# torognes/swarm

Hardware: AMD Instinct MI355X
Metric: amplicons/sec clustered (d=1) (higher is better)
Workload: dtype u64; 1 GPU; 10000000 synthetic amplicons x 150 bp, d=1 (10000000 per GPU; the metric's own size; configs[1]: configs1); per_gpu_queries=10000000, db_amplicons=10000000, step=swa_d1_index_build + swa_d1_network_device (B1 seam), db and CSR resident in HBM, route=streaming (d1_stream.inc), build=local, neighbour_links=17077441

## Files before the change

### swarm_amd/csrc/d1.hip

```cpp
#include "swa_internal.h"

#include <algorithm>
#include <type_traits>
#include <cstdlib>
#include <memory>
#include <thread>

namespace {

constexpr int kWaves = 4;
constexpr int kThreads = kWaves * 64;
constexpr int kQueueCap = 128;
constexpr uint32_t kEmpty = SWA_NO_AMPLICON;
constexpr size_t kMaxZobristLds = 96 * 1024;

struct alignas(16) swa_task {
  uint64_t hash;
  uint32_t heavy;
  uint32_t code;
};

struct NetArgs {
  const uint64_t * seqs;
  const uint64_t * seq_off;
// ... 748 lines not shown
  PartPlan p{};
  p.total = std::max(1u, total_bits);
  p.levels = (p.total + max_bits - 1) / max_bits;
  for (uint32_t l = 0; l < p.levels; ++l) { p.bits[l] = p.total / p.levels + (l < p.total % p.levels ? 1u : 0u); }
  return p;
}

struct PartJob {
  uint32_t nidx = 1;
  const unsigned long long * in[kMaxIdx] = {};
  unsigned long long * buf[kMaxIdx][2] = {};
  const uint64_t * cstart0[kMaxIdx] = {};
  uint64_t cstride0[kMaxIdx] = {};
  const uint32_t * csize0[kMaxIdx] = {};
  uint32_t csize_cap = 0, chunks0 = 1;
  bool single0 = true;
  uint64_t max_records = 0, max_tiles0 = 0;
  uint64_t out_cap = 0;
  uint32_t bias = 0, top_bit = 32;
  uint32_t tile = 4096;
  bool hist0_done = false;
  PartPlan plan{};
  uint32_t * out32[kMaxIdx] = {};
  uint32_t * cnt[kMaxIdx] = {}; uint32_t * ctile[kMaxIdx] = {}; uint64_t * starts[kMaxIdx] = {}; uint32_t * partial[kMaxIdx] = {};
  uint32_t * total[kMaxIdx] = {};
  uint64_t starts_stride = 0;
  const unsigned long long * out[kMaxIdx] = {}; const uint64_t * bstart[kMaxIdx] = {};
  uint32_t buckets = 0;
  int last = 0;
};

static void part_scratch(const PartJob & j, uint64_t * cnt, uint64_t * ctile, uint64_t * starts_half, uint64_t * partial) {
  uint64_t chunks = j.chunks0, c_max = 0, t_max = 0, s_max = 0;
  bool single = j.single0;
  for (uint32_t l = 0; l < j.plan.levels; ++l) {
    const uint64_t tiles = (l == 0 ? j.max_tiles0 : j.max_records / j.tile + chunks + 1);
    c_max = std::max(c_max, (tiles << j.plan.bits[l]) + 2);
    t_max = std::max(t_max, chunks + 2 + tiles + 2);
    chunks = (single ? 1 : chunks) << j.plan.bits[l];
    single = false;
    s_max = std::max(s_max, chunks + 2);
  }
  *cnt = c_max; *ctile = t_max; *starts_half = s_max; *partial = c_max / kFlatChunk + 2;
}

struct ClearList { uint32_t * p[8]; uint64_t words[8]; uint32_t n; };
__global__ __launch_bounds__(256) void k_clear_many(const ClearList c) {
  for (uint32_t k = 0; k < c.n; ++k) {
    for (uint64_t i = (uint64_t)blockIdx.x * blockDim.x + threadIdx.x; i < c.words[k]; i += (uint64_t)gridDim.x * blockDim.x) { c.p[k][i] = 0u; }
  }
}
static void clear_add(ClearList & c, void * p, uint64_t bytes) {
  c.p[c.n] = static_cast<uint32_t *>(p); c.words[c.n] = bytes / 4; ++c.n;
}
static int clear_launch(swa_ctx * ctx, const ClearList & c) {
  uint64_t most = 0;
  for (uint32_t k = 0; k < c.n; ++k) { most = std::max(most, c.words[k]); }
  if (c.n == 0 || most == 0) { return SWA_OK; }
  hipLaunchKernelGGL(k_clear_many, dim3(grid_for(ctx, most, 256, 8)), dim3(256), 0, ctx->stream, c);
  SWA_HIP(ctx, hipGetLastError());
  return SWA_OK;
}

static int run_partition(swa_ctx * ctx, PartJob & j) {
  uint64_t chunks = j.chunks0;
  bool single = j.single0;
  uint32_t used_bits = 0;
  const int cu_grid = ctx->num_cus * 8;
  for (uint32_t l = 0; l < j.plan.levels; ++l) {
    const uint32_t bits = j.plan.bits[l];
    used_bits += bits;
    const bool wide = bits > kPartMaxBits;
    const bool hist_done = l == 0 && j.hist0_done;
    const bool low_halves = l + 1 == j.plan.levels && j.out32[0] != nullptr;
    const bool have_form = wide ? (j.tile == 4096 || (j.tile == 8192 && hist_done)) && !low_halves
                                : (j.tile == 2048 && !low_halves) || j.tile == 4096;
    if (!have_form) { return swa_fail_msg(ctx, SWA_E_ARG, "partition: no kernel for this tile and bin count"); }
    PartArgs a{};
    a.single_seg = single ? 1u : 0u; a.bits = bits; a.shift = j.top_bit - used_bits; a.bias = j.bias; a.tile = j.tile;
    a.span = (single && l == 0 && chunks > 1 && j.tile == 4096 && !wide && !hist_done) ? 1u : 0u;
    const uint64_t tiles = (l == 0 ? j.max_tiles0 : j.max_records / j.tile + chunks + 1);
    a.run_bits = tiles >= (uint64_t)cu_grid ? 4u : 0u;
    for (uint32_t i = 0; i < j.nidx; ++i) {
      PartIdx & p = a.p[i];
      p.in = l == 0 ? j.in[i] : j.buf[i][(l - 1) & 1u];
      p.out = j.buf[i][l & 1u];
      p.out32 = low_halves ? j.out32[i] : nullptr;
      p.out_cap = j.out_cap;
      p.cstart = l == 0 ? j.cstart0[i] : j.starts[i] + ((l - 1) & 1u) * j.starts_stride;
      p.cstride = l == 0 ? j.cstride0[i] : 0;
      p.csize = l == 0 ? j.csize0[i] : nullptr;
      p.csize_cap = j.csize_cap;
      p.chunks = (uint32_t)chunks;
      p.ctile = j.ctile[i]; p.cnt = j.cnt[i];
      p.tchunk = j.ctile[i] + chunks + 1; p.tchunk_cap = (uint32_t)std::min<uint64_t>(tiles + 1, 0xFFFFFFFFu);
      p.next_start = j.starts[i] + (l & 1u) * j.starts_stride;
      p.total = j.total[i];
    }
    const dim3 grid_t((unsigned)((std::min<uint64_t>(std::max<uint64_t>(tiles, 1), (uint64_t)cu_grid) + 7) & ~7ull), j.nidx);
    if (chunks > 2048) { hipLaunchKernelGGL(k_part_tiles<1024>, dim3(1, j.nidx), dim3(1024), 0, ctx->stream, a); }
    else { hipLaunchKernelGGL(k_part_tiles<256>, dim3(1, j.nidx), dim3(256), 0, ctx->stream, a); }
    if (hist_done) {  }
    else if (wide) { hipLaunchKernelGGL((k_part_hist<1024, kPartTileMax, 256>), grid_t, dim3(256), 0, ctx->stream, a); }
    else if (a.span != 0u) { hipLaunchKernelGGL((k_part_hist<512, kPartTileMax, 256, true>), grid_t, dim3(256), 0, ctx->stream, a); }
    else { hipLaunchKernelGGL((k_part_hist<512, kPartTileMax, 256>), grid_t, dim3(256), 0, ctx->stream, a); }
    FlatScanArgs f{};
    f.unit_bits = bits;
    for (uint32_t i = 0; i < j.nidx; ++i) { f.v[i] = j.cnt[i]; f.units[i] = j.ctile[i] + chunks; f.partial[i] = j.partial[i]; f.total[i] = j.total[i]; }
    const dim3 grid_f((unsigned)std::min<uint64_t>(((tiles << bits) + 1 + kFlatChunk - 1) / kFlatChunk, (uint64_t)cu_grid), j.nidx);
    hipLaunchKernelGGL(k_flat_sums, grid_f, dim3(256), 0, ctx->stream, f);
    hipLaunchKernelGGL(k_flat_apply, grid_f, dim3(256), 0, ctx->stream, f);
    if (wide && j.tile == 8192) {
      constexpr size_t lds = part_scatter_lds(8192, 1024);
      if (!ctx->part_lds_opt_in) {
        SWA_HIP(ctx, hipFuncSetAttribute(reinterpret_cast<const void *>(&k_part_scatter<0, 8192, 1024, 1024>), hipFuncAttributeMaxDynamicSharedMemorySize, (int)lds));
        ctx->part_lds_opt_in = true;
      }
      hipLaunchKernelGGL((k_part_scatter<0, 8192, 1024, 1024>), grid_t, dim3(1024), lds, ctx->stream, a);
    }
    else if (wide) { hipLaunchKernelGGL((k_part_scatter<0, 4096, 1024, 512>), grid_t, dim3(512), part_scatter_lds(4096, 1024), ctx->stream, a); }
    else if (j.tile == 2048) { hipLaunchKernelGGL((k_part_scatter<0, 2048, 512, 512>), grid_t, dim3(512), part_scatter_lds(2048, 512), ctx->stream, a); }
    else if (a.span != 0u && low_halves) { hipLaunchKernelGGL((k_part_scatter<2, 4096, 512, 512, true>), grid_t, dim3(512), part_scatter_lds(4096, 512), ctx->stream, a); }
    else if (a.span != 0u) { hipLaunchKernelGGL((k_part_scatter<0, 4096, 512, 512, true>), grid_t, dim3(512), part_scatter_lds(4096, 512), ctx->stream, a); }
    else if (low_halves) { hipLaunchKernelGGL((k_part_scatter<2, 4096, 512, 512>), grid_t, dim3(512), part_scatter_lds(4096, 512), ctx->stream, a); }
    else { hipLaunchKernelGGL((k_part_scatter<0, 4096, 512, 512>), grid_t, dim3(512), part_scatter_lds(4096, 512), ctx->stream, a); }
    chunks = (single ? 1 : chunks) << bits;
    single = false;
    hipLaunchKernelGGL(k_part_starts, dim3((unsigned)std::min<uint64_t>((chunks + 256) / 256, (uint64_t)cu_grid), j.nidx), dim3(256), 0, ctx->stream, a);
    SWA_HIP(ctx, hipGetLastError());
  }
  j.buckets = (uint32_t)chunks;
  j.last = (int)((j.plan.levels - 1) & 1u);
  for (uint32_t i = 0; i < j.nidx; ++i) {
    j.out[i] = j.buf[i][j.last];
    j.bstart[i] = j.starts[i] + (uint64_t)j.last * j.starts_stride;
  }
  return SWA_OK;
}

static int ensure_lines(swa_ctx * ctx) {
  const uint32_t lq = line_quads_for(ctx);
  if (ctx->lines_ready && ctx->lines_quads == lq) { return SWA_OK; }
  const uint32_t n = ctx->db.n;
  SWA_TRY(swa_reserve(ctx, ctx->d_stream[kSbLines], (uint64_t)n * lq * 16u + 64u));
  auto * lines = static_cast<uint4 *>(ctx->d_stream[kSbLines].ptr);
  const auto * rank = static_cast<const uint32_t *>(ctx->d_arank.ptr);
  SWA_HIP(ctx, hipMemsetAsync(reinterpret_cast<uint8_t *>(lines) + (uint64_t)n * lq * 16u, 0, 64, ctx->stream));
  swa_t0(ctx, 15);
  const dim3 grid(grid_for(ctx, n, 256, 8));
  if (lq == 4u) { hipLaunchKernelGGL(k_lines_build<4>, grid, dim3(256), 0, ctx->stream, ctx->db.seqs, ctx->db.seq_off, ctx->db.seqlen, rank, n, lines); }
  else if (lq == 8u) { hipLaunchKernelGGL(k_lines_build<8>, grid, dim3(256), 0, ctx->stream, ctx->db.seqs, ctx->db.seq_off, ctx->db.seqlen, rank, n, lines); }
// ... 18 lines not shown
  const uint32_t lq = ctx->lines_quads;
  uint64_t item_room = 0;
  const ListRegions regions = list_regions(ctx, &item_room);
  const bool by_rec = ctx->route_rec[0] != nullptr;
  const bool routed = ctx->route_ids[0] != nullptr || by_rec;
  const uint64_t records = routed ? std::max<uint64_t>(std::max(ctx->route_m[0], ctx->route_m[1]), 1) : n;
  const uint32_t target = kG1Target, level_bits = 10u;
  uint32_t total_bits = 1;
  while ((records >> total_bits) > target && total_bits < 3 * kPartMaxBits) { ++total_bits; }
  total_bits = std::min<uint32_t>(total_bits + ctx->stream_extra_bits, 3 * kPartMaxBits);
  const bool keys_hist = !routed;
  PartJob j;
  j.nidx = 2;
  j.plan = total_bits <= level_bits ? plan_levels(total_bits, level_bits) : plan_levels(total_bits);
  j.max_records = records;
  j.out_cap = records + 1;
  const bool one_wide_level = total_bits > kPartMaxBits && j.plan.levels == 1;
  j.tile = one_wide_level ? (keys_hist ? 8192 : 4096) : 2048;
  j.max_tiles0 = records / j.tile + 2;
  j.chunks0 = 1; j.single0 = true; j.top_bit = 32; j.bias = 0;
  uint64_t e_cnt, e_tile, e_start, e_partial;
  part_scratch(j, &e_cnt, &e_tile, &e_start, &e_partial);
  const uint64_t buckets = 1ull << total_bits;
  e_partial = std::max<uint64_t>(e_partial, ((uint64_t)kListsPerIndex * buckets + 1) / kFlatChunk + 2);
  for (int i = 0; i < 2; ++i) {
    for (int h = 0; h < 2; ++h) { SWA_TRY(swa_reserve(ctx, ctx->d_stream[kSbRec + 2 * i + h], (records + 1) * sizeof(uint64_t))); }
    SWA_TRY(swa_reserve(ctx, ctx->d_stream[kSbCnt + i], e_cnt * sizeof(uint32_t)));
    SWA_TRY(swa_reserve(ctx, ctx->d_stream[kSbTile + i], e_tile * sizeof(uint32_t)));
    SWA_TRY(swa_reserve(ctx, ctx->d_stream[kSbStart + i], (2 * e_start + 4) * sizeof(uint64_t)));
    SWA_TRY(swa_reserve(ctx, ctx->d_stream[kSbPartial + i], e_partial * sizeof(uint32_t)));
    SWA_TRY(swa_reserve(ctx, ctx->d_stream[kSbMembers + i], (records + 1) * sizeof(uint32_t)));
    SWA_TRY(swa_reserve(ctx, ctx->d_stream[kSbKind + i], ((uint64_t)kListsPerIndex * buckets + 2) * sizeof(uint32_t)));
    SWA_TRY(swa_reserve(ctx, ctx->d_aitems[i], (item_room + 1) * sizeof(swa_item)));
  }
  SWA_TRY(swa_reserve(ctx, ctx->d_stream[kSbScal], 64 * sizeof(uint64_t)));
  SWA_TRY(swa_reserve(ctx, ctx->d_stream[kSbOver], ((uint64_t)n + 8) & ~3ull));
  SWA_TRY(swa_reserve(ctx, ctx->d_acounters, kCounterWords * sizeof(uint32_t)));
  {
    ClearList c{};
    clear_add(c, ctx->d_acounters.ptr, kCounterWords * sizeof(uint32_t));
    clear_add(c, ctx->d_guard.ptr, 8 * sizeof(uint64_t));
    clear_add(c, ctx->d_stream[kSbOver].ptr, ((uint64_t)n + 8) & ~3ull);
    for (int i = 0; i < 2; ++i) { clear_add(c, static_cast<uint32_t *>(ctx->d_stream[kSbKind + i].ptr) + (uint64_t)kListsPerIndex * buckets, sizeof(uint32_t)); }
    SWA_TRY(clear_launch(ctx, c));
  }
  swa_lap(ctx, "buffers reserved, counters cleared");
  auto * dflags = static_cast<uint32_t *>(ctx->d_flags.ptr);
  auto * scal = static_cast<uint64_t *>(ctx->d_stream[kSbScal].ptr);
  const uint32_t win_a = ctx->anchor_a, win_b = ctx->anchor_b;
  const uint32_t minlen = anchor_minlen(ctx), window_mode = (win_a != 0 || win_b != 0) ? 1u : 0u;

  KeyArgs k{};
  k.lines = static_cast<const uint4 *>(ctx->d_stream[kSbLines].ptr);
// ... 28 lines not shown
  else if (keys_hist) {
    const uint32_t ntiles = (uint32_t)((records + j.tile - 1) / j.tile);
    for (int i = 0; i < 2; ++i) { k.hist_cnt[i] = static_cast<uint32_t *>(ctx->d_stream[kSbCnt + i].ptr); }
    k.hist_bits = j.plan.bits[0]; k.hist_tile = j.tile; k.hist_ntiles = ntiles;
    k.hist_run_bits = j.max_tiles0 >= (uint64_t)ctx->num_cus * 8 ? 4u : 0u;
    const dim3 hgrid((unsigned)((std::min<uint64_t>(ntiles, (uint64_t)ctx->num_cus * 8) + 7) & ~7ull), 1u);
    hipLaunchKernelGGL(k_keys<true>, hgrid, dim3(256), 0, ctx->stream, k);
    j.hist0_done = true;
  } else {
    const dim3 kgrid((unsigned)grid_for(ctx, records, 256, 8), routed ? 2u : 1u);
    hipLaunchKernelGGL(k_keys<false>, kgrid, dim3(256), 0, ctx->stream, k);
  }
  swa_t1(ctx, 8);
  swa_lap(ctx, "k_keys");

  for (int i = 0; i < 2; ++i) {
    j.buf[i][0] = static_cast<unsigned long long *>(ctx->d_stream[kSbRec + 2 * i].ptr);
    j.buf[i][1] = static_cast<unsigned long long *>(ctx->d_stream[kSbRec + 2 * i + 1].ptr);
    j.in[i] = by_rec ? ctx->route_rec[i] : j.buf[i][1];
    j.cstart0[i] = nullptr; j.cstride0[i] = routed ? ctx->route_m[i] : n;
    j.cnt[i] = static_cast<uint32_t *>(ctx->d_stream[kSbCnt + i].ptr);
    j.ctile[i] = static_cast<uint32_t *>(ctx->d_stream[kSbTile + i].ptr);
    j.starts[i] = static_cast<uint64_t *>(ctx->d_stream[kSbStart + i].ptr);
    j.partial[i] = static_cast<uint32_t *>(ctx->d_stream[kSbPartial + i].ptr);
    j.total[i] = reinterpret_cast<uint32_t *>(scal + 8 + i);
  }
  j.starts_stride = e_start + 2;
  swa_t0(ctx, 9);
  SWA_TRY(run_partition(ctx, j));
  swa_t1(ctx, 9);
  swa_lap(ctx, "key partition");
  if (!ctx->guard_keys_done) {
    auto * gsum = static_cast<unsigned long long *>(ctx->d_guard.ptr) + 16;
    SWA_HIP(ctx, hipMemsetAsync(gsum, 0, 8 * sizeof(uint64_t), ctx->stream));
    GuardDbArgs gd{};
    gd.seqs = ctx->db.seqs; gd.seq_off = ctx->db.seq_off; gd.seqlen = ctx->db.seqlen; gd.n = n;
    for (int i = 0; i < 2; ++i) { gd.list[i] = k.list[i]; gd.list_count[i] = routed ? ctx->route_m[i] : 0; gd.list_rec[i] = by_rec ? ctx->route_rec[i] : nullptr; }
    gd.owner_rank = k.owner_rank; gd.owner_world = k.owner_world; gd.win_a = win_a; gd.win_b = win_b; gd.nwin = k.nwin;
    gd.out = gsum;
    hipLaunchKernelGGL(k_guard_db, dim3((unsigned)grid_for(ctx, records, 256, 8), routed ? 2u : 1u), dim3(256), 0, ctx->stream, gd);
    GuardRecArgs gr{};
    for (int i = 0; i < 2; ++i) { gr.rec[i] = j.out[i]; gr.total[i] = j.total[i]; }
    gr.out = gsum + 3;
    hipLaunchKernelGGL(k_guard_records, dim3((unsigned)grid_for(ctx, records, 256, 8), 2u), dim3(256), 0, ctx->stream, gr);
    ctx->guard_keys_pending = true;
  }

  swa_lap(ctx, "guard: second opinion");
  GroupArgs g{};
  for (int i = 0; i < 2; ++i) {
    GroupIdx & x = g.g[i];
    x.rec = const_cast<unsigned long long *>(j.out[i]);
    x.bstart = j.bstart[i];
    x.buckets = j.buckets;
    x.members = static_cast<uint32_t *>(ctx->d_stream[kSbMembers + i].ptr);
    x.items_tmp = j.buf[i][j.last ^ 1];
    x.kind_cnt = static_cast<uint32_t *>(ctx->d_stream[kSbKind + i].ptr);
  }
  g.pair_big = kPairBigCap; g.group_cap = kStreamGroupCap;
  g.flags = dflags;
  g.guard = static_cast<unsigned long long *>(ctx->d_guard.ptr);
  g.over = static_cast<uint8_t *>(ctx->d_stream[kSbOver].ptr);
  swa_t0(ctx, 10);
  {
    if (!ctx->g1_lds_opt_in) {
      SWA_HIP(ctx, hipFuncSetAttribute(reinterpret_cast<const void *>(&k_group1), hipFuncAttributeMaxDynamicSharedMemorySize, (int)kG1LdsBytes));
      ctx->g1_lds_opt_in = true;
    }
    hipLaunchKernelGGL(k_group1, dim3((unsigned)std::min<uint64_t>(buckets, (uint64_t)ctx->num_cus), 2), dim3(kG1Threads), kG1LdsBytes, ctx->stream, g);
  }
  swa_t1(ctx, 10);

  FlatScanArgs f{};
  ListArgs la{};
  auto * acounters = static_cast<uint32_t *>(ctx->d_acounters.ptr);
  for (int i = 0; i < 2; ++i) {
    f.v[i] = g.g[i].kind_cnt; f.units[i] = nullptr; f.fixed[i] = (uint64_t)kListsPerIndex * buckets + 1;
    f.partial[i] = j.partial[i]; f.total[i] = reinterpret_cast<uint32_t *>(scal + 10 + i);
    ListIdx & x = la.x[i];
    x.items_tmp = g.g[i].items_tmp; x.bstart = g.g[i].bstart; x.kind_pos = g.g[i].kind_cnt; x.buckets = (uint32_t)buckets;
    x.l.items = static_cast<swa_item *>(ctx->d_aitems[i].ptr);
    x.l.region = regions;
    x.l.counters = acounters + kCounterBase + (uint32_t)i * kWidthClasses * 8u;
    x.l.pair_big = g.pair_big;
  }
  const dim3 grid_k((unsigned)std::min<uint64_t>(((uint64_t)kListsPerIndex * buckets + kFlatChunk) / kFlatChunk, (uint64_t)ctx->num_cus * 8), 2);
  hipLaunchKernelGGL(k_flat_sums, grid_k, dim3(256), 0, ctx->stream, f);
  hipLaunchKernelGGL(k_flat_apply, grid_k, dim3(256), 0, ctx->stream, f);
  hipLaunchKernelGGL(k_group_lists, dim3((unsigned)std::min<uint64_t>((buckets + 3) / 4, (uint64_t)ctx->num_cus * 8), 2), dim3(256), 0, ctx->stream, la);
  SWA_HIP(ctx, hipGetLastError());
  swa_lap(ctx, "groups + work lists");
  ctx->list_regions_items = item_room;
  ctx->anchor_ready = true;
  ctx->stream_index = true;
  ctx->guard_index = true;
  return SWA_OK;
}

static int csr_from_chunks(swa_ctx * ctx, uint32_t first, uint32_t count, const unsigned long long * links, const uint64_t * d_cstart, uint64_t cstride,
                           const uint32_t * d_csize, uint32_t chunks, uint32_t csize_cap, uint64_t max_tiles0, uint64_t link_cap,
                           uint64_t * d_offsets, uint32_t * d_neighbours, uint64_t cap) {
  uint32_t nbits = 1;
  while (nbits < 32 && ((uint64_t)1 << nbits) < count) { ++nbits; }
  uint32_t r = std::min<uint32_t>(8, nbits - 1);
  if (nbits - r > 2 * kPartMaxBits) { r = std::min<uint32_t>(kCsrMaxR, nbits - 2 * kPartMaxBits); }
  PartJob j;
  j.nidx = 1;
  j.plan = plan_levels(nbits - r);
  j.max_records = link_cap;
  j.out_cap = link_cap;
  j.tile = 4096;
  j.max_tiles0 = max_tiles0;
  j.chunks0 = chunks; j.single0 = true; j.top_bit = nbits; j.bias = first;
  j.csize_cap = csize_cap;
  uint64_t e_cnt, e_tile, e_start, e_partial;
  part_scratch(j, &e_cnt, &e_tile, &e_start, &e_partial);
  SWA_TRY(swa_reserve(ctx, ctx->d_stream[kSbLinkA], (link_cap + 1) * sizeof(uint64_t)));
  SWA_TRY(swa_reserve(ctx, ctx->d_stream[kSbLinkB], (link_cap + 1) * sizeof(uint64_t)));
  SWA_TRY(swa_reserve(ctx, ctx->d_stream[kSbCnt], e_cnt * sizeof(uint32_t)));
  SWA_TRY(swa_reserve(ctx, ctx->d_stream[kSbTile], e_tile * sizeof(uint32_t)));
  SWA_TRY(swa_reserve(ctx, ctx->d_stream[kSbStart], (2 * e_start + 4) * sizeof(uint64_t)));
  SWA_TRY(swa_reserve(ctx, ctx->d_stream[kSbPartial], e_partial * sizeof(uint32_t)));
  SWA_TRY(swa_reserve(ctx, ctx->d_stream[kSbScal], 64 * sizeof(uint64_t)));
  j.in[0] = links;
  j.buf[0][0] = static_cast<unsigned long long *>(ctx->d_stream[kSbLinkA].ptr);
  j.buf[0][1] = static_cast<unsigned long long *>(ctx->d_stream[kSbLinkB].ptr);
  j.cstart0[0] = d_cstart; j.cstride0[0] = cstride;
  j.csize0[0] = d_csize;
  j.cnt[0] = static_cast<uint32_t *>(ctx->d_stream[kSbCnt].ptr);
  j.ctile[0] = static_cast<uint32_t *>(ctx->d_stream[kSbTile].ptr);
  j.starts[0] = static_cast<uint64_t *>(ctx->d_stream[kSbStart].ptr);
  j.partial[0] = static_cast<uint32_t *>(ctx->d_stream[kSbPartial].ptr);
  auto * extra = static_cast<uint64_t *>(ctx->d_status.ptr) + 48;
  j.total[0] = reinterpret_cast<uint32_t *>(extra + 1);
  j.starts_stride = e_start + 2;
  swa_t0(ctx, 13);
  SWA_TRY(run_partition(ctx, j));
  swa_t1(ctx, 13);
  CsrArgs c{};
  c.links = j.out[0]; c.bstart = j.bstart[0]; c.buckets = j.buckets; c.r = r; c.first = first; c.count = count;
  c.offsets = d_offsets; c.neighbours = d_neighbours; c.cap = d_neighbours != nullptr ? cap : 0;
  SWA_TRY(swa_reserve(ctx, ctx->d_stream[kSbHeavy], ((uint64_t)j.buckets + 2) * sizeof(uint32_t)));
  c.heavy = static_cast<uint32_t *>(ctx->d_stream[kSbHeavy].ptr) + 1;
  c.heavy_count = static_cast<uint32_t *>(ctx->d_stream[kSbHeavy].ptr);
  c.end_copy = extra;
  SWA_HIP(ctx, hipMemsetAsync(c.heavy_count, 0, sizeof(uint32_t), ctx->stream));
  swa_t0(ctx, 14);
  static const int csr_per_cu[2] = {
    [] { int nb = 0; return hipOccupancyMaxActiveBlocksPerMultiprocessor(&nb, k_csr_bucket<8>, 256, 0) == hipSuccess && nb > 0 ? nb : 4; }(),
    [] { int nb = 0; return hipOccupancyMaxActiveBlocksPerMultiprocessor(&nb, k_csr_bucket<9>, 256, 0) == hipSuccess && nb > 0 ? nb : 4; }() };
  const dim3 cgrid((unsigned)std::min<uint64_t>(((uint64_t)j.buckets + 3) / 4, (uint64_t)ctx->num_cus * (uint64_t)csr_per_cu[r <= 8 ? 0 : 1]));
  if (r <= 8) { hipLaunchKernelGGL(k_csr_bucket<8>, cgrid, dim3(256), 0, ctx->stream, c); }
  else { hipLaunchKernelGGL(k_csr_bucket<9>, cgrid, dim3(256), 0, ctx->stream, c); }
  hipLaunchKernelGGL(k_csr_bucket_big, dim3((unsigned)ctx->num_cus * 4), dim3(256), 0, ctx->stream, c);
  swa_t1(ctx, 14);
// ... 581 lines not shown
                         nseg, ctx->seg_cap, static_cast<const unsigned long long *>(ctx->d_seg_base.ptr), d_edge_list, cap);
    } else {
      stream_link_cap = std::max<uint64_t>(std::max<uint64_t>(cap, stream_link_cap), 2ull * count + 1024);
      SWA_TRY(launch_csr_stream(ctx, first, count, nseg, stream_link_cap, d_offsets, d_neighbours, cap));
    }
    SWA_HIP(ctx, hipGetLastError());
    swa_t1(ctx, 4);
    auto * status = static_cast<uint64_t *>(ctx->h_status);
    SWA_HIP(ctx, hipMemcpyAsync(status, ctx->d_status.ptr, 64 * sizeof(uint64_t), hipMemcpyDeviceToHost, ctx->stream));
    uint32_t * unserved_at = reinterpret_cast<uint32_t *>(status + 64);
    *unserved_at = 0;
    if (check_unserved) {
      SWA_HIP(ctx, hipMemcpyAsync(unserved_at, static_cast<uint32_t *>(ctx->d_acounters.ptr) + 2, sizeof(uint32_t), hipMemcpyDeviceToHost, ctx->stream));
    }
    SWA_HIP(ctx, hipStreamSynchronize(ctx->stream));
    const uint32_t unserved = *unserved_at;
    const uint64_t * got = status + 8 + 8;
    const uint64_t * guard = status + 24;
    const uint32_t anchor_overflow = reinterpret_cast<const uint32_t *>(status)[2];
    const uint64_t csr_end = status[48];
    const uint32_t links_sorted = (uint32_t)status[49];
    const bool guarded = ctx->anchor_usable;
    n_edges = got[0];
    if (guarded && anchor_overflow != 0) {
      ctx->stream_extra_bits = std::min<uint32_t>(ctx->stream_extra_bits + 2, 8);
      ctx->anchor_ready = false;
      continue;
    }
    if (check_unserved && unserved != 0) {
      SWA_TRY(ensure_full_index(ctx));
      continue;
    }
    if (d_edge_list == nullptr && got[1] <= ctx->seg_cap && n_edges > stream_link_cap) {
      stream_link_cap = n_edges + 1024;
      continue;
    }
    if (got[1] <= ctx->seg_cap) {
      clean = true;
      if (guarded) { SWA_TRY(guard_check(ctx, guard, got)); }
      if (d_edge_list == nullptr) { SWA_TRY(csr_check(ctx, csr_end, links_sorted, n_edges)); }
      twins = guarded && reinterpret_cast<const uint32_t *>(status)[0] != 0u;
      break;
    }
    while (ctx->seg_cap < 2 * got[1]) { ctx->seg_cap <<= 1; }
  }
  if (!clean) {
// ... 565 lines not shown
```

### swarm_amd/csrc/d1_stream.inc

```

constexpr uint32_t kPartTileMax = 4096;
constexpr uint32_t kPartMaxBits = 9;
constexpr unsigned long long kRecAbsent = ~0ull;
constexpr uint32_t kMaxIdx = 2;
constexpr uint32_t kStreamGroupCap = 4096;

template <int LQ>
__global__ __launch_bounds__(256) void k_lines_build(const uint64_t * __restrict__ seqs, const uint64_t * __restrict__ seq_off,
                                                     const uint32_t * __restrict__ seqlen, const uint32_t * __restrict__ rank, uint32_t n,
                                                     uint4 * __restrict__ lines) {
  constexpr uint32_t C = 2u * LQ - 1u;
  for (uint32_t i = blockIdx.x * blockDim.x + threadIdx.x; i < n; i += gridDim.x * blockDim.x) {
    const uint32_t len = seqlen[i];
    const uint64_t * s = seqs + seq_off[i];
    const uint32_t nw = (len + 31u) >> 5;
    uint32_t d[4 * LQ];
    d[0] = len; d[1] = rank[i];
#pragma unroll
    for (uint32_t k = 0; k < C; ++k) {
      const uint64_t w = k < nw ? s[k] : 0ull;
      d[2 + 2 * k] = (uint32_t)w; d[3 + 2 * k] = (uint32_t)(w >> 32);
    }
#pragma unroll
    for (uint32_t q = 0; q < (uint32_t)LQ; ++q) { lines[(uint64_t)i * LQ + q] = make_uint4(d[4 * q], d[4 * q + 1], d[4 * q + 2], d[4 * q + 3]); }
// ... 234 lines not shown
__global__ __launch_bounds__(256) void k_guard_records(const GuardRecArgs a) {
  const uint32_t which = blockIdx.y, m = *a.total[which];
  unsigned long long sum = 0ull;
  for (uint32_t e = blockIdx.x * blockDim.x + threadIdx.x; e < m; e += gridDim.x * blockDim.x) { sum += mix64(a.rec[which][e]); }
  guard_reduce(sum, a.out + which);
}

struct PartIdx {
  const unsigned long long * in;
  unsigned long long * out;
  uint32_t * out32;
  uint64_t out_cap;
  const uint64_t * cstart;
  uint64_t cstride;
  const uint32_t * csize;
  uint32_t csize_cap;
  uint32_t chunks;
  uint32_t * ctile;
  uint32_t * tchunk;
  uint32_t tchunk_cap;
  uint32_t * cnt;
  uint64_t * next_start;
  uint32_t * total;
};
struct PartArgs {
  PartIdx p[kMaxIdx];
  uint32_t single_seg;
  uint32_t shift, bits;
  uint32_t bias;
  uint32_t tile;
  uint32_t run_bits;
  uint32_t span;
};

__device__ __forceinline__ uint32_t part_chunk_size(const PartIdx & p, uint32_t c) {
  if (p.csize != nullptr) { return min(p.csize[c], p.csize_cap); }
  return p.cstart != nullptr ? (uint32_t)(p.cstart[c + 1] - p.cstart[c]) : (uint32_t)p.cstride;
}

template <uint32_t THREADS> __device__ __forceinline__ uint64_t block_exclusive_scan_of(uint64_t v, uint64_t * smem, uint64_t & total);
template <uint32_t THREADS>
__global__ __launch_bounds__(THREADS) void k_part_tiles(const PartArgs a) {
  __shared__ uint64_t smem[THREADS / 64u];
  const PartIdx & p = a.p[blockIdx.y];
  uint64_t carry = 0;
  const bool tile_pow2 = (a.tile & (a.tile - 1u)) == 0u;
  const uint32_t tile_shift = 31u - (uint32_t)__clz((int)a.tile);
  for (uint32_t base = 0; base < p.chunks; base += 8u * THREADS) {
    uint32_t v[8];
    uint64_t mine = 0;
#pragma unroll
    for (uint32_t k = 0; k < 8u; ++k) {
      const uint32_t c = base + threadIdx.x * 8u + k;
      v[k] = c < p.chunks ? (a.span != 0u ? part_chunk_size(p, c) : (part_chunk_size(p, c) + a.tile - 1u) / a.tile) : 0u;
    }
#pragma unroll
    for (uint32_t k = 0; k < 8u; ++k) { mine += v[k]; }
    uint64_t total;
    uint64_t run = carry + block_exclusive_scan_of<THREADS>(mine, smem, total);
#pragma unroll
    for (uint32_t k = 0; k < 8u; ++k) {
      const uint32_t c = base + threadIdx.x * 8u + k;
      if (c < p.chunks) {
        p.ctile[c] = (uint32_t)run;
        if (v[k] != 0u && a.span != 0u) {
          const uint32_t r32 = (uint32_t)run;
          const uint32_t first = tile_pow2 ? (r32 + a.tile - 1u) >> tile_shift : (r32 + a.tile - 1u) / a.tile;
// ... 112 lines not shown
    const uint32_t t = xcd_tile(v, a.run_bits);
    if (t >= ntiles) { continue; }
    for (uint32_t b = threadIdx.x; b < bins; b += THREADS) { hist[b] = 0u; }
    PartTile tile{0u, 0u, 0ull};
    const auto count_one = [&](unsigned long long r) {
      if (r != kRecAbsent) { atomicAdd(&hist[(((uint32_t)(r >> 32) - a.bias) >> a.shift) & (bins - 1u)], 1u); }
    };
    if constexpr (SPAN) {
      (void)part_span<TILE / THREADS, THREADS>(p, a.tile, t, span, [&](uint32_t, uint64_t place) { count_one(p.in[place]); });
    } else {
      tile = part_tile(p, a.tile, t, sh);
#pragma unroll
      for (uint32_t k = 0; k < TILE / THREADS; ++k) {
        const uint32_t j = k * THREADS + threadIdx.x;
        if (j < tile.count) { count_one(p.in[tile.first + j]); }
      }
    }
    __syncthreads();
    for (uint32_t b = threadIdx.x; b < bins; b += THREADS) { p.cnt[part_flat(a, p, tile.c, t, b)] = hist[b]; }
    __syncthreads();
  }
}

constexpr uint32_t kFlatChunk = 4096;
constexpr uint32_t kFlatPer = kFlatChunk / 256u;
struct FlatScanArgs { uint32_t * v[kMaxIdx]; const uint32_t * units[kMaxIdx]; uint32_t unit_bits; uint64_t fixed[kMaxIdx]; uint32_t * partial[kMaxIdx]; uint32_t * total[kMaxIdx]; };
__device__ __forceinline__ uint64_t flat_length(const FlatScanArgs & a, uint32_t i) {
  return a.units[i] != nullptr ? ((uint64_t)*a.units[i] << a.unit_bits) + 1u : a.fixed[i];
}

__global__ __launch_bounds__(256) void k_flat_sums(const FlatScanArgs a) {
  __shared__ uint64_t smem[4];
  const uint32_t * v = a.v[blockIdx.y];
  const uint64_t m = flat_length(a, blockIdx.y);
  for (uint64_t blk = blockIdx.x; blk * kFlatChunk < m; blk += gridDim.x) {
    const uint64_t base = blk * kFlatChunk + (uint64_t)threadIdx.x * kFlatPer;
    uint64_t s = 0;
#pragma unroll
    for (uint32_t k = 0; k < kFlatPer; ++k) { if (base + k < m) { s += v[base + k]; } }
    uint64_t total;
    (void)block_exclusive_scan(s, smem, total);
    if (threadIdx.x == 0) { a.partial[blockIdx.y][blk] = (uint32_t)total; }
  }
}

__global__ __launch_bounds__(256) void k_flat_apply(const FlatScanArgs a) {
  __shared__ uint64_t smem[4];
  uint32_t * v = a.v[blockIdx.y];
  const uint64_t m = flat_length(a, blockIdx.y);
  const uint32_t * partial = a.partial[blockIdx.y];
  const uint64_t nblk = (m + kFlatChunk - 1) / kFlatChunk;
  for (uint64_t blk = blockIdx.x; blk < nblk; blk += gridDim.x) {
    uint64_t before = 0;
    for (uint64_t q = threadIdx.x; q < blk; q += 256u) { before += partial[q]; }
    uint64_t prefix;
    (void)block_exclusive_scan(before, smem, prefix);
    const uint64_t base = blk * kFlatChunk + (uint64_t)threadIdx.x * kFlatPer;
    uint32_t c[kFlatPer];
    uint64_t s = 0;
#pragma unroll
    for (uint32_t k = 0; k < kFlatPer; ++k) { c[k] = base + k < m ? v[base + k] : 0u; s += c[k]; }
    uint64_t total;
    uint64_t run = prefix + block_exclusive_scan(s, smem, total);
#pragma unroll
    for (uint32_t k = 0; k < kFlatPer; ++k) { if (base + k < m) { v[base + k] = (uint32_t)run; } run += c[k]; }
    if (blk + 1 == nblk && threadIdx.x == 0) { *a.total[blockIdx.y] = (uint32_t)(prefix + total); }
  }
}

template <uint32_t THREADS>
__device__ __forceinline__ uint64_t block_exclusive_scan_of(uint64_t v, uint64_t * smem, uint64_t & total) {
  const uint32_t lane = threadIdx.x & 63u, wave = threadIdx.x >> 6;
  uint64_t incl = v;
#pragma unroll
  for (unsigned d = 1; d < 64; d <<= 1) { const uint64_t t = swa_shfl_up_u64(incl, d); if (lane >= d) { incl += t; } }
  if (lane == 63u) { smem[wave] = incl; }
  __syncthreads();
  uint64_t wave_off = 0, tot = 0;
#pragma unroll
  for (uint32_t w = 0; w < THREADS / 64u; ++w) { const uint64_t x = smem[w]; wave_off += w < wave ? x : 0ull; tot += x; }
  __syncthreads();
  total = tot;
  return wave_off + incl - v;
}

template <int MODE, uint32_t TILE, uint32_t BINS, uint32_t THREADS, bool SPAN = false>
__global__ __launch_bounds__(THREADS) __attribute__((amdgpu_waves_per_eu(SPAN && THREADS == 512 ? 8 : 1))) void k_part_scatter(const PartArgs a) {
  constexpr uint32_t kPartPer = TILE / THREADS;
  extern __shared__ __attribute__((aligned(16))) unsigned long long part_lds[];
// ... 56 lines not shown
        stage[at] = rec[k];
      }
    }
    __syncthreads();
    const uint32_t present = lstart[bins - 1u] + hist[bins - 1u];
#pragma unroll
    for (uint32_t k = 0; k < kPartPer; ++k) {
      const uint32_t j = k * THREADS + threadIdx.x;
      if (j < present) {
        const unsigned long long r = stage[j];
        const uint32_t d = (((uint32_t)(r >> 32) - a.bias) >> a.shift) & (bins - 1u);
        const uint64_t g = (uint64_t)goff[d] + (j - lstart[d]);
        if (g < p.out_cap) {
          if (MODE == 2) { p.out32[g] = (uint32_t)r; } else { p.out[g] = r; }
        }
      }
    }
    __syncthreads();
  }
}

constexpr size_t part_scatter_lds(uint32_t tile, uint32_t bins) { return (size_t)tile * 8u + 3u * (size_t)bins * 4u; }

__global__ __launch_bounds__(256) void k_part_starts(const PartArgs a) {
  const PartIdx & p = a.p[blockIdx.y];
  const uint32_t segs = a.single_seg != 0u ? 1u : p.chunks;
  const uint64_t buckets = (uint64_t)segs << a.bits;
  for (uint64_t i = (uint64_t)blockIdx.x * blockDim.x + threadIdx.x; i <= buckets; i += (uint64_t)gridDim.x * blockDim.x) {
    if (i == buckets) { p.next_start[i] = *p.total; continue; }
    const uint32_t c = (uint32_t)(i >> a.bits), b = (uint32_t)i & ((1u << a.bits) - 1u);
    p.next_start[i] = p.cnt[a.single_seg != 0u ? (uint64_t)b * p.ctile[p.chunks] : ((uint64_t)p.ctile[c] << a.bits) + (uint64_t)b * (p.ctile[c + 1] - p.ctile[c])];
  }
}

struct GroupIdx {
  unsigned long long * rec;
  const uint64_t * bstart;
  uint32_t buckets;
  uint32_t * members;
  unsigned long long * items_tmp;
  uint32_t * kind_cnt;
};
struct GroupArgs {
  GroupIdx g[kMaxIdx];
  uint32_t pair_big, group_cap;
  uint32_t * flags;
  unsigned long long * guard;
  uint8_t * over;
};

constexpr uint32_t kG1Threads = 1024;
constexpr uint32_t kG1SlotBits = 13, kG1Slots = 1u << kG1SlotBits;
constexpr uint32_t kG1DupBits = 14, kG1DupSlots = 1u << kG1DupBits;
constexpr uint32_t kG1Target = 10240;
constexpr size_t kG1LdsBytes = kG1Slots * 4 * 2 + kG1DupSlots * 4;
static_assert(kG1Slots * 4 <= kG1DupSlots * 4, "the groups' places lie in the area behind the two tables");
constexpr uint32_t kG1OverBit = 0x80000000u;

constexpr uint32_t kG1Per = 8;
constexpr uint32_t kG1Tail = 2;

__device__ __forceinline__ uint32_t g1_size(uint32_t w) { return w & 0xFFFFu; }
__device__ __forceinline__ uint32_t g1_class(uint32_t w) {
  const uint32_t bits = (w >> 16) & 0x1Fu;
  return bits == 0u ? 0u : 31u - (uint32_t)__clz((int)bits);
}
__device__ __forceinline__ bool g1_over(uint32_t w, uint32_t cap) { return g1_size(w) > 1u && (g1_size(w) > cap || g1_class(w) >= kTooLong); }
__device__ __forceinline__ uint32_t g1_list(uint32_t w, uint32_t pair_big, uint32_t cap) {
  const uint32_t g = g1_size(w);
  if (g < 2u || g1_over(w, cap)) { return kListsPerIndex; }
  const uint32_t kind = g <= kSeedsPerItem ? pair_class(g) : (g <= pair_big ? kPairClasses : kPairClasses + 1u);
// ... 94 lines not shown
    if ((int)lane >= d) { x += up; }
  }
  const unsigned long long tot = lane_value64(x, 15);
  const unsigned long long before = wave == 0u ? 0ull : lane_value64(x, (int)wave - 1);
  __syncthreads();
  total = tot;
  return before + incl - v;
}

__global__ __launch_bounds__(kG1Threads) void k_group1(const GroupArgs a) {
  extern __shared__ uint32_t g1_lds[];
  uint32_t * tcnt = g1_lds;
  uint32_t * tkey = tcnt + kG1Slots;
  uint32_t * toff = tkey + kG1Slots + (kG1DupSlots - kG1Slots);
  uint32_t * staged = tkey;
  __shared__ uint32_t kcnt[kListsPerIndex], kbase[kListsPerIndex];
  __shared__ unsigned long long smem16[16];
  __shared__ uint32_t sh_fail;
  __shared__ uint32_t gsum[3];
  uint32_t * glist = tkey;
  const uint32_t which = blockIdx.y;
  const GroupIdx & g = a.g[which];
  if (threadIdx.x < 3u) { gsum[threadIdx.x] = 0u; }
  for (uint32_t b = blockIdx.x; b < g.buckets; b += gridDim.x) {
    uint32_t tid = threadIdx.x;
    asm volatile("" : "+v"(tid));
    const uint32_t lane = tid & 63u;
    const uint64_t start = g.bstart[b];
    const uint32_t c = (uint32_t)(g.bstart[b + 1] - start);
    if (c == 0u) {
      if (tid < kListsPerIndex) { g.kind_cnt[tid * g.buckets + b] = 0u; }
      continue;
    }
    if (c > 0xFFFEu) {
      for (uint32_t r = tid; r < c; r += kG1Threads) {
        const uint32_t id = (uint32_t)g.rec[start + r];
        g.members[start + r] = id;
        atomicOr(reinterpret_cast<unsigned int *>(a.over + (id & ~3u)), (1u << which) << (8u * (id & 3u)));
      }
      if (tid < kListsPerIndex) { g.kind_cnt[tid * g.buckets + b] = 0u; }
      if (tid == 0) { atomicOr(a.flags + 4, 1u); atomicAdd(a.flags + 5, c); atomicAdd(a.guard + 6u + which, (unsigned long long)c); }
      continue;
    }
    const uint32_t cap = a.group_cap;
    uint32_t rkey[kG1Per], rid[kG1Per];
    uint32_t here = 0u;
// ... 502 lines not shown
```

Before: 5.998 billion amplicons/s.

## Replace two-pass flat scan with single-pass decoupled look-back scan fused with bucket starts

Replaces the k_flat_sums + k_flat_apply pair with one k_flat_scan kernel. It takes chunk indices from an atomic counter, publishes aggregate and inclusive flags, and looks back across earlier chunks one wavefront at a time. The same kernel also writes the next-level bucket start offsets from LDS, so the separate k_part_starts launch is removed. Scan state is widened to 64-bit status words and zeroed inside the preceding kernels. A spin bound reports stalls through a status word that the host checks. This cuts kernel launches and a full re-read of the counts per partition level. The cost is inter-block spinning, which depends on forward progress, plus some extra complexity.

```diff
diff --git a/swarm_amd/csrc/d1.hip b/swarm_amd/csrc/d1.hip
--- a/swarm_amd/csrc/d1.hip
+++ b/swarm_amd/csrc/d1.hip
@@ -794,13 +794,17 @@
   bool hist0_done = false;
   PartPlan plan{};
   uint32_t * out32[kMaxIdx] = {};
-  uint32_t * cnt[kMaxIdx] = {}; uint32_t * ctile[kMaxIdx] = {}; uint64_t * starts[kMaxIdx] = {}; uint32_t * partial[kMaxIdx] = {};
+  uint32_t * cnt[kMaxIdx] = {}; uint32_t * ctile[kMaxIdx] = {}; uint64_t * starts[kMaxIdx] = {};
+  unsigned long long * partial[kMaxIdx] = {};
   uint32_t * total[kMaxIdx] = {};
   uint64_t starts_stride = 0;
   const unsigned long long * out[kMaxIdx] = {}; const uint64_t * bstart[kMaxIdx] = {};
   uint32_t buckets = 0;
   int last = 0;
 };
+
+constexpr uint32_t kScanStallWord = 50;
+static unsigned long long * scan_stall_word(swa_ctx * ctx) { return static_cast<unsigned long long *>(ctx->d_status.ptr) + kScanStallWord; }
 
 static void part_scratch(const PartJob & j, uint64_t * cnt, uint64_t * ctile, uint64_t * starts_half, uint64_t * partial) {
   uint64_t chunks = j.chunks0, c_max = 0, t_max = 0, s_max = 0;
@@ -813,7 +817,7 @@
     single = false;
     s_max = std::max(s_max, chunks + 2);
   }
-  *cnt = c_max; *ctile = t_max; *starts_half = s_max; *partial = c_max / kFlatChunk + 2;
+  *cnt = c_max; *ctile = t_max; *starts_half = s_max; *partial = flat_state_words(c_max);
 }
 
 struct ClearList { uint32_t * p[8]; uint64_t words[8]; uint32_t n; };
@@ -853,6 +857,7 @@
     a.span = (single && l == 0 && chunks > 1 && j.tile == 4096 && !wide && !hist_done) ? 1u : 0u;
     const uint64_t tiles = (l == 0 ? j.max_tiles0 : j.max_records / j.tile + chunks + 1);
     a.run_bits = tiles >= (uint64_t)cu_grid ? 4u : 0u;
+    a.scan_words = (uint32_t)flat_state_words((tiles << bits) + 1);
     for (uint32_t i = 0; i < j.nidx; ++i) {
       PartIdx & p = a.p[i];
       p.in = l == 0 ? j.in[i] : j.buf[i][(l - 1) & 1u];
@@ -868,6 +873,7 @@
       p.tchunk = j.ctile[i] + chunks + 1; p.tchunk_cap = (uint32_t)std::min<uint64_t>(tiles + 1, 0xFFFFFFFFu);
       p.next_start = j.starts[i] + (l & 1u) * j.starts_stride;
       p.total = j.total[i];
+      p.scan_state = j.partial[i];
     }
     const dim3 grid_t((unsigned)((std::min<uint64_t>(std::max<uint64_t>(tiles, 1), (uint64_t)cu_grid) + 7) & ~7ull), j.nidx);
     if (chunks > 2048) { hipLaunchKernelGGL(k_part_tiles<1024>, dim3(1, j.nidx), dim3(1024), 0, ctx->stream, a); }
@@ -877,11 +883,13 @@
     else if (a.span != 0u) { hipLaunchKernelGGL((k_part_hist<512, kPartTileMax, 256, true>), grid_t, dim3(256), 0, ctx->stream, a); }
     else { hipLaunchKernelGGL((k_part_hist<512, kPartTileMax, 256>), grid_t, dim3(256), 0, ctx->stream, a); }
     FlatScanArgs f{};
-    f.unit_bits = bits;
-    for (uint32_t i = 0; i < j.nidx; ++i) { f.v[i] = j.cnt[i]; f.units[i] = j.ctile[i] + chunks; f.partial[i] = j.partial[i]; f.total[i] = j.total[i]; }
+    f.unit_bits = bits; f.single_seg = a.single_seg; f.stall = scan_stall_word(ctx);
+    for (uint32_t i = 0; i < j.nidx; ++i) {
+      f.v[i] = j.cnt[i]; f.units[i] = j.ctile[i] + chunks; f.partial[i] = j.partial[i]; f.total[i] = j.total[i];
+      f.next_start[i] = a.p[i].next_start; f.ctile[i] = j.ctile[i]; f.chunks[i] = (uint32_t)chunks;
+    }
     const dim3 grid_f((unsigned)std::min<uint64_t>(((tiles << bits) + 1 + kFlatChunk - 1) / kFlatChunk, (uint64_t)cu_grid), j.nidx);
-    hipLaunchKernelGGL(k_flat_sums, grid_f, dim3(256), 0, ctx->stream, f);
-    hipLaunchKernelGGL(k_flat_apply, grid_f, dim3(256), 0, ctx->stream, f);
+    hipLaunchKernelGGL(k_flat_scan, grid_f, dim3(kFlatThreads), 0, ctx->stream, f);
     if (wide && j.tile == 8192) {
       constexpr size_t lds = part_scatter_lds(8192, 1024);
       if (!ctx->part_lds_opt_in) {
@@ -898,7 +906,6 @@
     else { hipLaunchKernelGGL((k_part_scatter<0, 4096, 512, 512>), grid_t, dim3(512), part_scatter_lds(4096, 512), ctx->stream, a); }
     chunks = (single ? 1 : chunks) << bits;
     single = false;
-    hipLaunchKernelGGL(k_part_starts, dim3((unsigned)std::min<uint64_t>((chunks + 256) / 256, (uint64_t)cu_grid), j.nidx), dim3(256), 0, ctx->stream, a);
     SWA_HIP(ctx, hipGetLastError());
   }
   j.buckets = (uint32_t)chunks;
@@ -963,13 +970,13 @@
   uint64_t e_cnt, e_tile, e_start, e_partial;
   part_scratch(j, &e_cnt, &e_tile, &e_start, &e_partial);
   const uint64_t buckets = 1ull << total_bits;
-  e_partial = std::max<uint64_t>(e_partial, ((uint64_t)kListsPerIndex * buckets + 1) / kFlatChunk + 2);
+  e_partial = std::max<uint64_t>(e_partial, flat_state_words((uint64_t)kListsPerIndex * buckets + 1));
   for (int i = 0; i < 2; ++i) {
     for (int h = 0; h < 2; ++h) { SWA_TRY(swa_reserve(ctx, ctx->d_stream[kSbRec + 2 * i + h], (records + 1) * sizeof(uint64_t))); }
     SWA_TRY(swa_reserve(ctx, ctx->d_stream[kSbCnt + i], e_cnt * sizeof(uint32_t)));
     SWA_TRY(swa_reserve(ctx, ctx->d_stream[kSbTile + i], e_tile * sizeof(uint32_t)));
     SWA_TRY(swa_reserve(ctx, ctx->d_stream[kSbStart + i], (2 * e_start + 4) * sizeof(uint64_t)));
-    SWA_TRY(swa_reserve(ctx, ctx->d_stream[kSbPartial + i], e_partial * sizeof(uint32_t)));
+    SWA_TRY(swa_reserve(ctx, ctx->d_stream[kSbPartial + i], e_partial * sizeof(uint64_t)));
     SWA_TRY(swa_reserve(ctx, ctx->d_stream[kSbMembers + i], (records + 1) * sizeof(uint32_t)));
     SWA_TRY(swa_reserve(ctx, ctx->d_stream[kSbKind + i], ((uint64_t)kListsPerIndex * buckets + 2) * sizeof(uint32_t)));
     SWA_TRY(swa_reserve(ctx, ctx->d_aitems[i], (item_room + 1) * sizeof(swa_item)));
@@ -1044,7 +1051,7 @@
     j.cnt[i] = static_cast<uint32_t *>(ctx->d_stream[kSbCnt + i].ptr);
     j.ctile[i] = static_cast<uint32_t *>(ctx->d_stream[kSbTile + i].ptr);
     j.starts[i] = static_cast<uint64_t *>(ctx->d_stream[kSbStart + i].ptr);
-    j.partial[i] = static_cast<uint32_t *>(ctx->d_stream[kSbPartial + i].ptr);
+    j.partial[i] = static_cast<unsigned long long *>(ctx->d_stream[kSbPartial + i].ptr);
     j.total[i] = reinterpret_cast<uint32_t *>(scal + 8 + i);
   }
   j.starts_stride = e_start + 2;
@@ -1078,7 +1085,9 @@
     x.members = static_cast<uint32_t *>(ctx->d_stream[kSbMembers + i].ptr);
     x.items_tmp = j.buf[i][j.last ^ 1];
     x.kind_cnt = static_cast<uint32_t *>(ctx->d_stream[kSbKind + i].ptr);
-  }
+    x.scan_state = j.partial[i];
+  }
+  g.scan_words = (uint32_t)flat_state_words((uint64_t)kListsPerIndex * buckets + 1);
   g.pair_big = kPairBigCap; g.group_cap = kStreamGroupCap;
   g.flags = dflags;
   g.guard = static_cast<unsigned long long *>(ctx->d_guard.ptr);
@@ -1107,8 +1116,8 @@
     x.l.pair_big = g.pair_big;
   }
   const dim3 grid_k((unsigned)std::min<uint64_t>(((uint64_t)kListsPerIndex * buckets + kFlatChunk) / kFlatChunk, (uint64_t)ctx->num_cus * 8), 2);
-  hipLaunchKernelGGL(k_flat_sums, grid_k, dim3(256), 0, ctx->stream, f);
-  hipLaunchKernelGGL(k_flat_apply, grid_k, dim3(256), 0, ctx->stream, f);
+  f.stall = scan_stall_word(ctx);
+  hipLaunchKernelGGL(k_flat_scan, grid_k, dim3(kFlatThreads), 0, ctx->stream, f);
   hipLaunchKernelGGL(k_group_lists, dim3((unsigned)std::min<uint64_t>((buckets + 3) / 4, (uint64_t)ctx->num_cus * 8), 2), dim3(256), 0, ctx->stream, la);
   SWA_HIP(ctx, hipGetLastError());
   swa_lap(ctx, "groups + work lists");
@@ -1142,7 +1151,7 @@
   SWA_TRY(swa_reserve(ctx, ctx->d_stream[kSbCnt], e_cnt * sizeof(uint32_t)));
   SWA_TRY(swa_reserve(ctx, ctx->d_stream[kSbTile], e_tile * sizeof(uint32_t)));
   SWA_TRY(swa_reserve(ctx, ctx->d_stream[kSbStart], (2 * e_start + 4) * sizeof(uint64_t)));
-  SWA_TRY(swa_reserve(ctx, ctx->d_stream[kSbPartial], e_partial * sizeof(uint32_t)));
+  SWA_TRY(swa_reserve(ctx, ctx->d_stream[kSbPartial], e_partial * sizeof(uint64_t)));
   SWA_TRY(swa_reserve(ctx, ctx->d_stream[kSbScal], 64 * sizeof(uint64_t)));
   j.in[0] = links;
   j.buf[0][0] = static_cast<unsigned long long *>(ctx->d_stream[kSbLinkA].ptr);
@@ -1152,7 +1161,7 @@
   j.cnt[0] = static_cast<uint32_t *>(ctx->d_stream[kSbCnt].ptr);
   j.ctile[0] = static_cast<uint32_t *>(ctx->d_stream[kSbTile].ptr);
   j.starts[0] = static_cast<uint64_t *>(ctx->d_stream[kSbStart].ptr);
-  j.partial[0] = static_cast<uint32_t *>(ctx->d_stream[kSbPartial].ptr);
+  j.partial[0] = static_cast<unsigned long long *>(ctx->d_stream[kSbPartial].ptr);
   auto * extra = static_cast<uint64_t *>(ctx->d_status.ptr) + 48;
   j.total[0] = reinterpret_cast<uint32_t *>(extra + 1);
   j.starts_stride = e_start + 2;
@@ -1780,6 +1789,10 @@
     const uint32_t links_sorted = (uint32_t)status[49];
     const bool guarded = ctx->anchor_usable;
     n_edges = got[0];
+    if (status[kScanStallWord] != 0) {
+      SWA_HIP(ctx, hipMemsetAsync(scan_stall_word(ctx), 0, sizeof(uint64_t), ctx->stream));
+      return swa_fail_msg(ctx, SWA_E_INTERNAL, "d=1: a partition scan waited beyond its bound for the chunks before it");
+    }
     if (guarded && anchor_overflow != 0) {
       ctx->stream_extra_bits = std::min<uint32_t>(ctx->stream_extra_bits + 2, 8);
       ctx->anchor_ready = false;
diff --git a/swarm_amd/csrc/d1_stream.inc b/swarm_amd/csrc/d1_stream.inc
--- a/swarm_amd/csrc/d1_stream.inc
+++ b/swarm_amd/csrc/d1_stream.inc
@@ -280,6 +280,7 @@
   uint32_t * cnt;
   uint64_t * next_start;
   uint32_t * total;
+  unsigned long long * scan_state;
 };
 struct PartArgs {
   PartIdx p[kMaxIdx];
@@ -289,6 +290,7 @@
   uint32_t tile;
   uint32_t run_bits;
   uint32_t span;
+  uint32_t scan_words;
 };
 
 __device__ __forceinline__ uint32_t part_chunk_size(const PartIdx & p, uint32_t c) {
@@ -301,6 +303,7 @@
 __global__ __launch_bounds__(THREADS) void k_part_tiles(const PartArgs a) {
   __shared__ uint64_t smem[THREADS / 64u];
   const PartIdx & p = a.p[blockIdx.y];
+  for (uint32_t i = threadIdx.x; i < a.scan_words; i += THREADS) { p.scan_state[i] = 0ull; }
   uint64_t carry = 0;
   const bool tile_pow2 = (a.tile & (a.tile - 1u)) == 0u;
   const uint32_t tile_shift = 31u - (uint32_t)__clz((int)a.tile);
@@ -459,49 +462,132 @@
   }
 }
 
-constexpr uint32_t kFlatChunk = 4096;
-constexpr uint32_t kFlatPer = kFlatChunk / 256u;
-struct FlatScanArgs { uint32_t * v[kMaxIdx]; const uint32_t * units[kMaxIdx]; uint32_t unit_bits; uint64_t fixed[kMaxIdx]; uint32_t * partial[kMaxIdx]; uint32_t * total[kMaxIdx]; };
+constexpr uint32_t kFlatChunk = 8192;
+constexpr uint32_t kFlatThreads = 512;
+constexpr uint32_t kFlatPer = kFlatChunk / kFlatThreads;
+struct FlatScanArgs {
+  uint32_t * v[kMaxIdx]; const uint32_t * units[kMaxIdx]; uint32_t unit_bits; uint64_t fixed[kMaxIdx];
+  unsigned long long * partial[kMaxIdx];
+  uint32_t * total[kMaxIdx];
+  uint64_t * next_start[kMaxIdx]; const uint32_t * ctile[kMaxIdx]; uint32_t chunks[kMaxIdx]; uint32_t single_seg;
+  unsigned long long * stall;
+};
 __device__ __forceinline__ uint64_t flat_length(const FlatScanArgs & a, uint32_t i) {
   return a.units[i] != nullptr ? ((uint64_t)*a.units[i] << a.unit_bits) + 1u : a.fixed[i];
 }
-
-__global__ __launch_bounds__(256) void k_flat_sums(const FlatScanArgs a) {
-  __shared__ uint64_t smem[4];
-  const uint32_t * v = a.v[blockIdx.y];
-  const uint64_t m = flat_length(a, blockIdx.y);
-  for (uint64_t blk = blockIdx.x; blk * kFlatChunk < m; blk += gridDim.x) {
-    const uint64_t base = blk * kFlatChunk + (uint64_t)threadIdx.x * kFlatPer;
-    uint64_t s = 0;
-#pragma unroll
-    for (uint32_t k = 0; k < kFlatPer; ++k) { if (base + k < m) { s += v[base + k]; } }
-    uint64_t total;
-    (void)block_exclusive_scan(s, smem, total);
-    if (threadIdx.x == 0) { a.partial[blockIdx.y][blk] = (uint32_t)total; }
-  }
-}
-
-__global__ __launch_bounds__(256) void k_flat_apply(const FlatScanArgs a) {
-  __shared__ uint64_t smem[4];
-  uint32_t * v = a.v[blockIdx.y];
-  const uint64_t m = flat_length(a, blockIdx.y);
-  const uint32_t * partial = a.partial[blockIdx.y];
+constexpr uint64_t flat_state_words(uint64_t entries) { return (entries + kFlatChunk - 1) / kFlatChunk + 1; }
+
+typedef __attribute__((address_space(1))) unsigned long long flat_gu64;
+typedef __attribute__((address_space(1))) uint32_t flat_gu32;
+constexpr unsigned long long kScanAgg = 1ull << 32;
+constexpr unsigned long long kScanIncl = 2ull << 32;
+constexpr uint32_t kScanSpins = 1u << 22;
+
+__device__ __forceinline__ uint64_t flat_buckets_below(const FlatScanArgs & a, uint32_t y, uint64_t x) {
+  const uint32_t * ctile = a.ctile[y];
+  const uint32_t chunks = a.chunks[y], bits = a.unit_bits;
+  if (a.single_seg != 0u) {
+    const uint64_t tiles = ctile[chunks], most = (1ull << bits) + 1u;
+    if (tiles == 0u) { return x > 0u ? most : 0u; }
+    return min((x + tiles - 1u) / tiles, most);
+  }
+  const uint32_t lane = threadIdx.x & 63u;
+  uint32_t lo = 0, hi = chunks + 1u;
+  while (lo < hi) {
+    const uint32_t step = (hi - lo + 63u) / 64u, q = lo + (lane + 1u) * step - 1u;
+    const bool at_or_above = q < hi && ((uint64_t)ctile[q] << bits) >= x;
+    const unsigned long long m = __ballot(at_or_above);
+    if (m == 0ull) { lo += min(64u, (hi - lo) / step) * step; continue; }
+    const uint32_t k = (uint32_t)__ffsll((long long)m) - 1u;
+    hi = lo + (k + 1u) * step - 1u;
+    lo = k == 0u ? lo : lo + k * step;
+  }
+  if (lo == chunks + 1u) { return ((uint64_t)chunks << bits) + 1u; }
+  if (lo == 0u) { return 0u; }
+  const uint32_t c = lo - 1u, t0 = ctile[c], nt = ctile[lo] - t0;
+  const uint64_t first = (uint64_t)t0 << bits, all = 1ull << bits;
+  const uint64_t below = nt == 0u ? all : min(all, (x - first + nt - 1u) / nt);
+  return ((uint64_t)c << bits) + below;
+}
+
+__global__ __launch_bounds__(kFlatThreads) void k_flat_scan(const FlatScanArgs a) {
+  __shared__ uint64_t smem[kFlatThreads / 64u];
+  __shared__ uint32_t vals[kFlatChunk];
+  __shared__ uint64_t sh_range[2];
+  __shared__ uint32_t sh_blk, sh_prefix;
+  const uint32_t y = blockIdx.y, lane = threadIdx.x & 63u, wave = threadIdx.x >> 6;
+  uint32_t * v = a.v[y];
+  const uint64_t m = flat_length(a, y);
   const uint64_t nblk = (m + kFlatChunk - 1) / kFlatChunk;
-  for (uint64_t blk = blockIdx.x; blk < nblk; blk += gridDim.x) {
-    uint64_t before = 0;
-    for (uint64_t q = threadIdx.x; q < blk; q += 256u) { before += partial[q]; }
-    uint64_t prefix;
-    (void)block_exclusive_scan(before, smem, prefix);
-    const uint64_t base = blk * kFlatChunk + (uint64_t)threadIdx.x * kFlatPer;
+  flat_gu64 * status = (flat_gu64 *)(a.partial[y]) + 1;
+  const bool starts = a.next_start[y] != nullptr;
+  for (;;) {
+    if (threadIdx.x == 0) { sh_blk = __hip_atomic_fetch_add((flat_gu32 *)(a.partial[y]), 1u, __ATOMIC_RELAXED, __HIP_MEMORY_SCOPE_AGENT); }
+    __syncthreads();
+    const uint64_t blk = sh_blk;
+    if (blk >= nblk) { return; }
+    const uint64_t lo = blk * kFlatChunk, base = lo + (uint64_t)threadIdx.x * kFlatPer;
     uint32_t c[kFlatPer];
     uint64_t s = 0;
 #pragma unroll
     for (uint32_t k = 0; k < kFlatPer; ++k) { c[k] = base + k < m ? v[base + k] : 0u; s += c[k]; }
-    uint64_t total;
-    uint64_t run = prefix + block_exclusive_scan(s, smem, total);
-#pragma unroll
-    for (uint32_t k = 0; k < kFlatPer; ++k) { if (base + k < m) { v[base + k] = (uint32_t)run; } run += c[k]; }
-    if (blk + 1 == nblk && threadIdx.x == 0) { *a.total[blockIdx.y] = (uint32_t)(prefix + total); }
+    uint64_t agg;
+    const uint64_t run = block_exclusive_scan_of<kFlatThreads>(s, smem, agg);
+    if (wave == 0u) {
+      uint32_t prefix = 0;
+      if (blk == 0u) {
+        if (lane == 0u) { __hip_atomic_store(status, kScanIncl | (uint32_t)agg, __ATOMIC_RELAXED, __HIP_MEMORY_SCOPE_AGENT); }
+      } else {
+        if (lane == 0u) { __hip_atomic_store(status + blk, kScanAgg | (uint32_t)agg, __ATOMIC_RELAXED, __HIP_MEMORY_SCOPE_AGENT); }
+        int64_t end = (int64_t)blk - 1;
+        for (uint32_t spins = 0;;) {
+          const int64_t q = end - (int64_t)lane;
+          const unsigned long long w = q >= 0 ? __hip_atomic_load(status + q, __ATOMIC_RELAXED, __HIP_MEMORY_SCOPE_AGENT) : kScanIncl;
+          if (!__all((w >> 32) != 0ull)) {
+            if (++spins < kScanSpins) { __builtin_amdgcn_s_sleep(1); continue; }
+            if (lane == 0u) { atomicAdd(a.stall, 1ull); }
+            break;
+          }
+          const unsigned long long incl = __ballot((w >> 32) == 2ull);
+          const uint32_t upto = incl != 0ull ? (uint32_t)__ffsll((long long)incl) - 1u : 63u;
+          uint32_t x = lane <= upto ? (uint32_t)w : 0u;
+#pragma unroll
+          for (int o = 32; o > 0; o >>= 1) { x += (uint32_t)__shfl_xor((int)x, o, 64); }
+          prefix += x;
+          if (incl != 0ull) { break; }
+          end -= 64;
+        }
+        if (lane == 0u) { __hip_atomic_store(status + blk, kScanIncl | (uint32_t)(prefix + (uint32_t)agg), __ATOMIC_RELAXED, __HIP_MEMORY_SCOPE_AGENT); }
+      }
+      if (lane == 0u) { sh_prefix = prefix; }
+    } else if (starts && wave <= 2u) {
+      const uint64_t r = flat_buckets_below(a, y, wave == 1u ? lo : min(lo + kFlatChunk, m));
+      if (lane == 0u) { sh_range[wave - 1u] = r; }
+    }
+    __syncthreads();
+    uint32_t at = sh_prefix + (uint32_t)run;
+#pragma unroll
+    for (uint32_t k = 0; k < kFlatPer; ++k) {
+      if (base + k < m) { v[base + k] = at; }
+      if (starts) { vals[threadIdx.x * kFlatPer + k] = at; }
+      at += c[k];
+    }
+    if (blk + 1 == nblk && threadIdx.x == 0) { *a.total[y] = sh_prefix + (uint32_t)agg; }
+    if (starts) {
+      __syncthreads();
+      const uint32_t * ctile = a.ctile[y];
+      const uint32_t chunks = a.chunks[y], bits = a.unit_bits;
+      for (uint64_t i = sh_range[0] + threadIdx.x; i < sh_range[1]; i += kFlatThreads) {
+        uint64_t e;
+        if (a.single_seg != 0u) { e = i * ctile[chunks]; }
+        else {
+          const uint32_t cc = (uint32_t)(i >> bits), b = (uint32_t)i & ((1u << bits) - 1u);
+          e = cc == chunks ? (uint64_t)ctile[chunks] << bits : ((uint64_t)ctile[cc] << bits) + (uint64_t)b * (ctile[cc + 1] - ctile[cc]);
+        }
+        a.next_start[y][i] = vals[e - lo];
+      }
+    }
+    __syncthreads();
   }
 }
 
@@ -604,17 +690,6 @@
 
 constexpr size_t part_scatter_lds(uint32_t tile, uint32_t bins) { return (size_t)tile * 8u + 3u * (size_t)bins * 4u; }
 
-__global__ __launch_bounds__(256) void k_part_starts(const PartArgs a) {
-  const PartIdx & p = a.p[blockIdx.y];
-  const uint32_t segs = a.single_seg != 0u ? 1u : p.chunks;
-  const uint64_t buckets = (uint64_t)segs << a.bits;
-  for (uint64_t i = (uint64_t)blockIdx.x * blockDim.x + threadIdx.x; i <= buckets; i += (uint64_t)gridDim.x * blockDim.x) {
-    if (i == buckets) { p.next_start[i] = *p.total; continue; }
-    const uint32_t c = (uint32_t)(i >> a.bits), b = (uint32_t)i & ((1u << a.bits) - 1u);
-    p.next_start[i] = p.cnt[a.single_seg != 0u ? (uint64_t)b * p.ctile[p.chunks] : ((uint64_t)p.ctile[c] << a.bits) + (uint64_t)b * (p.ctile[c + 1] - p.ctile[c])];
-  }
-}
-
 struct GroupIdx {
   unsigned long long * rec;
   const uint64_t * bstart;
@@ -622,6 +697,7 @@
   uint32_t * members;
   unsigned long long * items_tmp;
   uint32_t * kind_cnt;
+  unsigned long long * scan_state;
 };
 struct GroupArgs {
   GroupIdx g[kMaxIdx];
@@ -629,6 +705,7 @@
   uint32_t * flags;
   unsigned long long * guard;
   uint8_t * over;
+  uint32_t scan_words;
 };
 
 constexpr uint32_t kG1Threads = 1024;
@@ -769,6 +846,7 @@
   const uint32_t which = blockIdx.y;
   const GroupIdx & g = a.g[which];
   if (threadIdx.x < 3u) { gsum[threadIdx.x] = 0u; }
+  if (blockIdx.x == 0u) { for (uint32_t i = threadIdx.x; i < a.scan_words; i += kG1Threads) { g.scan_state[i] = 0ull; } }
   for (uint32_t b = blockIdx.x; b < g.buckets; b += gridDim.x) {
     uint32_t tid = threadIdx.x;
     asm volatile("" : "+v"(tid));
```

Result: no change. 5.992 billion amplicons/s, median of 2 (-0.1%).
